# tspooner/rsrl

Hardware: AMD Instinct MI355X
Metric: env-steps/sec (whole node), MountainCar Q-learning Fourier-5 (higher is better)
Workload: dtype f32

## Files before the change

### rsrl_amd/csrc/abi_ctx.hip

```cpp
#include "ctx.hpp"

thread_local std::string g_last_error;

int fail(int code, const char* fmt, ...) {
    char buf[512];
    va_list ap; va_start(ap, fmt); vsnprintf(buf, sizeof(buf), fmt, ap); va_end(ap);
    g_last_error = buf;
    if (code == RSRL_HIP_EHIP || code == RSRL_HIP_ENOMEM) (void)hipGetLastError();
    return code;
}

static Switches read_switches() {
    Switches sw;
    sw.no_graph = getenv("RSRL_NO_GRAPH") != nullptr;
    sw.no_persist = getenv("RSRL_NO_PERSIST") != nullptr;
    sw.no_trait_defer = getenv("RSRL_NO_TRAIT_DEFER") != nullptr;
    sw.k1_feature_major = getenv("RSRL_K1_FEATURE_MAJOR") != nullptr;
    if (const char* e = getenv("RSRL_K1_QUAD")) sw.k1_quad = e[0] != '0' ? 1 : 0;
    if (const char* e = getenv("RSRL_SPARSE_CHUNK")) { const int v = atoi(e); sw.sparse_chunk = v > 0 && v < 16 ? 16 : v; }
    if (const char* e = getenv("RSRL_PEER_TIMEOUT_MS")) sw.peer_timeout_ms = atol(e);
    if (const char* e = getenv("RSRL_WAVE_PK")) sw.no_wave_pk = e[0] == '0';
    if (const char* e = getenv("RSRL_REG_PRODUCER")) sw.no_reg_producer = e[0] == '0';
    return sw;
}
bool no_coalesce_switch() { return getenv("RSRL_NO_COALESCE") != nullptr; }

static AgentFamily classify(const rsrl_hip_config& cfg, size_t w_elems) {
    using F = AgentFamily;
    const bool fourier = cfg.basis == RSRL_FOURIER, tile = cfg.basis == RSRL_TILE_CODING;
    const bool wave = is_wave(cfg), reg = is_reg_fourier(cfg);
    const int al = cfg.algo;
    if (cfg.domain == RSRL_HIV_TREATMENT) return F::Hiv;
    if (is_ac(al)) return F::AcReg;
    if (is_tdac(al)) return F::TdAcReg;
    if (is_reinforce(al)) return F::ReinforceReg;
    if (is_lstd(al)) return F::LstdReg;
    if (is_tdac_lstd(al)) return F::TdAcLstdReg;
    if (cfg.weight_mode == RSRL_W_SHARED) return fourier ? F::SharedDense : (is_sparse_lambda(cfg) ? F::SharedSparseLambda : F::SharedTile);
    if (wave && is_wave_aux_algo(al)) return F::WaveAux;
    if (is_pred(al)) return tile ? F::TdTile : (reg ? F::TdReg : F::TdGeneric);
    if (al == RSRL_Q_SIGMA) return wave ? F::WaveQSigma : (reg ? F::QSigmaReg : F::QSigmaGeneric);
    if (al == RSRL_GREEDY_GQ) return reg ? F::GqReg : F::GqGeneric;
    if (is_lambda(al)) return tile ? F::LambdaTile : (wave ? F::WaveLambda : (reg ? F::LambdaReg : F::LambdaGeneric));
    if (wave) return F::WaveControl;
    if (reg) return cfg.steps_per_launch == 1 && (uint64_t)w_elems * 4ull < (1ull << 32) ? F::RegStep : F::RegFused;
    return F::Generic;
}
static const char* train_kernel_name(const rsrl_hip_ctx* c) {
    if (c->family == AgentFamily::WaveControl && c->cfg.weight_dtype == RSRL_W_BF16 && !c->sw.no_wave_pk) return "k_train_wave_pk";
    if (c->family == AgentFamily::RegStep && c->w_ls != 1) return c->k1_quad ? "k_step_reg_q4" : "k_step_reg_lm";
    return family_row(c).kernel;
}
static size_t stat_slots(Slots geometry, int64_t N, int F) {
    switch (geometry) {
    case Slots::Block: return grid_for(N);
// ... 155 lines not shown
    TRY(check_config(*cfg));
    c->cfg = *cfg;
    c->D = kDomainShape[cfg->domain][0]; c->A = kDomainShape[cfg->domain][1];
    c->F = 1;
    for (int i = 0; i < c->D; ++i) c->F *= cfg->basis == RSRL_FOURIER ? cfg->order + 1 : cfg->tiles_per_dim;
    if (cfg->basis == RSRL_TILE_CODING) c->F *= cfg->n_tilings;
    int ndev = 0;
    HIP_TRY(hipGetDeviceCount(&ndev));
    if (ndev < 1) return fail(RSRL_HIP_EHIP, "no HIP device");
    if (cfg->device < 0 || cfg->device >= ndev) return fail(RSRL_HIP_EINVAL, "device %d out of range (%d devices)", cfg->device, ndev);
    HIP_TRY(hipSetDevice(cfg->device));
    { int cus = 0; HIP_TRY(hipDeviceGetAttribute(&cus, hipDeviceAttributeMultiprocessorCount, cfg->device)); if (cus > 0) { c->n_simd = 4 * cus; c->n_cu = cus; } }
    if (cfg->peer_timeout_ms < 0) return fail(RSRL_HIP_EINVAL, "peer_timeout_ms must be >= 0");
    c->sw = read_switches();
    if (cfg->peer_timeout_ms > 0) c->peer_timeout = (uint64_t)cfg->peer_timeout_ms * 100000ull;
    else if (c->sw.peer_timeout_ms > 0) c->peer_timeout = (uint64_t)c->sw.peer_timeout_ms * 100000ull;
    if (cfg->stream) { c->stream = (hipStream_t)cfg->stream; c->own_stream = false; }
    else { HIP_TRY(hipStreamCreateWithFlags(&c->stream, hipStreamNonBlocking)); c->own_stream = true; }
    const int64_t N = cfg->n_envs;
    const bool shared = cfg->weight_mode == RSRL_W_SHARED;
    c->w_stride = shared ? 1 : N;
    const AlgoRow& agent = kAlgo[cfg->algo];
    c->Aw = agent.v ? 1 : c->A;
    c->w_elems = (size_t)c->Aw * c->F * (size_t)(shared ? 1 : N);
    c->family = classify(*cfg, c->w_elems);
    if (c->family == AgentFamily::RegStep && (c->A * c->F) % 4 == 0 && c->F % 4 == 0 && !c->sw.k1_feature_major) {
        c->w_stride = 1;
        c->w_ls = (int64_t)c->A * c->F;
        c->k1_quad = c->A <= 3 && (c->sw.k1_quad >= 0 ? c->sw.k1_quad == 1 : N >= 131072);
    }
    if (c->family == AgentFamily::RegFused && !c->sw.no_reg_producer && cfg->epsilon_decay == 1.0 && N <= (int64_t)kBlock * c->n_cu) {
        int lds = 0;
        HIP_TRY(hipDeviceGetAttribute(&lds, hipDeviceAttributeMaxSharedMemoryPerBlock, cfg->device));
        c->reg_producer = train_reg_pw_serves(cfg->domain, cfg->order, cfg->algo, lds);
    }
    c->train_kernel = train_kernel_name(c);
    c->dw_elems = (size_t)c->Aw * c->F;
    c->n_stat_slots = stat_slots(c->k1_quad ? Slots::Block64 : family_row(c).slots, N, c->F);
    TRY(ctx_alloc(c, &c->state, sizeof(float) * c->D * (size_t)N));
    TRY(ctx_alloc(c, &c->action, sizeof(int32_t) * (size_t)N));
    TRY(ctx_alloc(c, &c->ep_step, sizeof(uint32_t) * (size_t)N));
    c->w_bytes = c->w_elems * (cfg->weight_dtype == RSRL_W_BF16 ? 2 : 4);
    TRY(ctx_alloc(c, &c->W, c->w_bytes));
    TRY(ctx_alloc(c, &c->dW, sizeof(float) * c->dw_elems));
    TRY(ctx_alloc(c, &c->qcache, sizeof(float) * c->A * (size_t)N));
    if (cfg->domain == RSRL_HIV_TREATMENT) TRY(ctx_alloc(c, &c->hiv_y, sizeof(double) * 6 * (size_t)N));
    if (c->w_ls != 1 && cfg->weight_dtype == RSRL_W_F32 && cfg->epsilon_decay == 1.0 && trait_lm_available(cfg->domain, cfg->order, cfg->algo)) {
        TRY(ctx_alloc(c, &c->tq_key, sizeof(float) * c->D * (size_t)N));
        TRY(ctx_alloc(c, &c->tq_q, sizeof(float) * c->A * (size_t)N));
    }
    if (cfg->algo == RSRL_Q_SIGMA) {
        TRY(ctx_alloc(c, &c->qs_buf, sizeof(float) * (size_t)(c->D + 5) * (size_t)cfg->n_steps * (size_t)N, true));
        TRY(ctx_alloc(c, &c->qs_head, sizeof(uint32_t) * (size_t)N, true));
        TRY(ctx_alloc(c, &c->qs_len, sizeof(uint32_t) * (size_t)N, true));
    }
    if (cfg->epsilon_decay != 1.0) {
        TRY(ctx_alloc(c, &c->eps, sizeof(float) * (size_t)N));
        hipLaunchKernelGGL(k_fill_f32, dim3(grid_for(N)), dim3(kBlock), 0, c->stream, c->eps, N, (float)cfg->epsilon);
        KCHECK();
    }
    if (c->family == AgentFamily::SharedSparseLambda) {
        const int64_t slice = (int64_t)(c->F / cfg->n_tilings) * c->A;
        if (slice > 65536) return fail(RSRL_HIP_EINVAL, "SARSALambda / QLambda over a shared tile table: one tiling's slice (cells * actions = %lld entries) must not "
                                                        "exceed 65 536 (16-bit slice-relative keys between the step and the trace kernel)", (long long)slice);
        TRY(ctx_alloc(c, &c->sp_len, sizeof(uint32_t) * (size_t)cfg->n_tilings * (size_t)N, true));
        TRY(ctx_alloc(c, &c->sp_keys, sizeof(uint16_t) * (size_t)kSparseCap * (size_t)N, true));
        TRY(ctx_alloc(c, &c->sp_vals, sizeof(float) * (size_t)kSparseCap * (size_t)N, true));
// ... 285 lines not shown
```

### rsrl_amd/csrc/abi_train.hip

```cpp
#include "ctx.hpp"

RSRL_DEFINE_FX_READER(fx_saturations_train)

int timing_begin(rsrl_hip_ctx* c) {
    if (!c->timing) return RSRL_HIP_OK;
    if (c->events_used == c->events.size()) {
        hipEvent_t a, b;
        HIP_TRY(hipEventCreate(&a)); HIP_TRY(hipEventCreate(&b));
        c->events.emplace_back(a, b);
    }
    HIP_TRY(hipEventRecord(c->events[c->events_used].first, c->stream));
    return RSRL_HIP_OK;
}
int timing_end(rsrl_hip_ctx* c, uint32_t launches) {
    if (!c->timing) return RSRL_HIP_OK;
    HIP_TRY(hipEventRecord(c->events[c->events_used].second, c->stream));
    if (c->event_launches.size() <= c->events_used) c->event_launches.resize(c->events_used + 1);
    c->event_launches[c->events_used] = launches;
    c->events_used++;
    return RSRL_HIP_OK;
}

static inline int fold_in_step(const rsrl_hip_ctx* c) { return !c->multi ? 1 : (c->cfg.exchange == RSRL_EXCHANGE_PEER ? 0 : 1); }
static inline long long* tab_set_of(const rsrl_hip_ctx* c, uint64_t t) { return c->sh_tab + (size_t)kTabRep * c->dw_elems * (size_t)(t % 3u); }
// ... 268 lines not shown
    const dim3 grid(grid_for(io ? io->M : k.n_envs)), block(kBlock);
    const bool td_lambda = cf.algo == RSRL_TD_LAMBDA;
    bool ok = true;
    switch (c->family) {
    case AgentFamily::WaveAux: case AgentFamily::WaveQSigma: case AgentFamily::WaveLambda:
        launch_wave_agent(c, k, t, chunk, d_stats, io); break;
    case AgentFamily::TdTile: ok = launch_td_tile(cf.domain, cf.n_tilings, td_lambda, c->stream, k, g, make_td(c), t, chunk, d_stats, io); break;
    case AgentFamily::TdGeneric: ok = launch_td_model(cf, grid, block, c->stream, k, make_td(c), g, td_lambda, t, chunk, d_stats, io); break;
    case AgentFamily::TdReg: ok = launch_td(cf.domain, cf.order, td_lambda, grid, block, c->stream, k, make_td(c), t, chunk, d_stats, io); break;
    case AgentFamily::QSigmaReg: ok = launch_qsigma(cf.domain, cf.order, grid, block, c->stream, k, make_qs(c), g, t, chunk, d_stats, io); break;
    case AgentFamily::QSigmaGeneric: ok = launch_qsigma_model(cf, grid, block, c->stream, k, make_qs(c), g, t, chunk, d_stats, io); break;
    case AgentFamily::GqReg: ok = launch_gq(cf.domain, cf.order, cf.policy, grid, block, c->stream, k, make_gq(c), t, chunk, d_stats, io); break;
    case AgentFamily::GqGeneric: ok = launch_gq_model(cf, grid, block, c->stream, k, make_gq(c), g, t, chunk, d_stats, io); break;
    case AgentFamily::LambdaTile: ok = launch_lambda_tile(cf.domain, cf.n_tilings, c->stream, k, g, make_lambda(c), t, chunk, d_stats, io); break;
    case AgentFamily::LambdaGeneric: ok = launch_lambda_model(cf, grid, block, c->stream, k, make_lambda(c), g, t, chunk, d_stats, io); break;
    case AgentFamily::LambdaReg: ok = launch_lambda(cf.domain, cf.order, cf.algo, cf.policy, grid, block, c->stream, k, make_lambda(c), t, chunk, d_stats, io); break;
    case AgentFamily::WaveControl:
        for_wave(c, [&](auto tag) {
            using T = decltype(tag); using WT = typename T::wt;
            const dim3 wg(wave_grid_for(k.n_envs));
            if constexpr (WaveIO<WT>::kBf16) {
                if (!c->sw.no_wave_pk) {
                    if (k.eps) hipLaunchKernelGGL((k_train_wave_pk<T::domain, true>), wg, block, 0, c->stream, k, (WT*)c->W, t, chunk, d_stats);
                    else hipLaunchKernelGGL((k_train_wave_pk<T::domain>), wg, block, 0, c->stream, k, (WT*)c->W, t, chunk, d_stats);
                    return;
                }
            }
            if (k.eps) hipLaunchKernelGGL((k_train_wave<T::domain, WT, true>), wg, block, 0, c->stream, k, (WT*)c->W, t, chunk, d_stats);
            else hipLaunchKernelGGL((k_train_wave<T::domain, WT>), wg, block, 0, c->stream, k, (WT*)c->W, t, chunk, d_stats);
        });
        break;
    case AgentFamily::RegStep: return enqueue_k1_step(c, k, d_stats, t, nullptr);
    case AgentFamily::RegFused:
        if (c->reg_producer && !k.eps) { ok = launch_train_reg_pw(cf.algo, cf.policy, grid, c->stream, k, t, chunk, d_stats); break; }
        ok = launch_train_reg(cf.domain, cf.order, cf.algo, cf.policy, grid, block, c->stream, k, t, chunk, d_stats);
        break;
    case AgentFamily::Generic:
        ok = for_model(c, [&](auto tag) {
            using M = typename decltype(tag)::type;
            hipLaunchKernelGGL((k_train_mem<M>), grid, block, 0, c->stream, k, g, t, chunk, d_stats);
        });
        break;
    case AgentFamily::Hiv:
        if (io) launch_hiv_handle(c->stream, k, g, *io, t);
        else launch_hiv_train(c->stream, k, g, c->hiv_y, t, chunk, d_stats);
        break;
    case AgentFamily::AcReg:
        ok = launch_ac(cf.domain, cf.order, cf.algo == RSRL_Q_ACTOR_CRITIC ? AC_CRITIC_Q : AC_CRITIC_ADVANTAGE, grid, block, c->stream, k, c->Z, t, chunk, d_stats, io);
        break;
    case AgentFamily::TdAcReg: ok = launch_tdac(cf.domain, cf.order, grid, block, c->stream, k, c->Z, t, chunk, d_stats, io); break;
    case AgentFamily::LstdReg: ok = launch_lstd(cf.domain, cf.order, cf.algo == RSRL_ILSTD, c->stream, k, make_lstd(c), t, chunk, d_stats, io); break;
    case AgentFamily::TdAcLstdReg: ok = launch_tdac_lstd(cf.domain, cf.order, c->stream, k, make_tdac_lstd(c), t, chunk, d_stats, io); break;
    case AgentFamily::ReinforceReg:
        ok = !io && launch_reinforce(cf.domain, cf.order, cf.algo == RSRL_BASELINE_REINFORCE, grid, block, c->stream, k, make_reinforce(c), t, chunk, d_stats, nullptr);
        break;
    default: ok = false; break;
    }
    if (!ok) return NO_MODEL(c);
    KCHECK();
    return RSRL_HIP_OK;
}

int train_now(rsrl_hip_ctx* c, int64_t n_steps, rsrl_hip_stats* stats_out) {
    HIP_TRY(hipSetDevice(c->cfg.device));
    c->tq_valid = false;
    DevStats* d_stats = stats_out ? c->d_stats : nullptr;
    if (d_stats) HIP_TRY(hipMemsetAsync(c->d_stats, 0, sizeof(DevStats) * c->n_stat_slots, c->stream));
// ... 182 lines not shown
```

### rsrl_amd/csrc/ctx.hpp

```cpp
#pragma once
#include <hip/hip_runtime.h>
#include <rccl/rccl.h>

#include <cmath>
#include <cstdarg>
#include <cstdio>
#include <cstring>
#include <unistd.h>
#include <dlfcn.h>
#include <map>
#include <mutex>
#include <string>
#include <vector>

#include "../../include/rsrl_hip.h"
#pragma GCC visibility push(hidden)
#define RSRL_API_BEGIN _Pragma("GCC visibility push(default)") extern "C" {
#define RSRL_API_END } _Pragma("GCC visibility pop")
#include "launch.hpp"
#include "models.hpp"
#include "model_list.hpp"
#include "kernels_wave.hpp"
#include "kernels_lambda.hpp"
#include "kernels_gq.hpp"
// ... 147 lines not shown
    {AgentFamily::GqGeneric, "k_train_gq_mem", 256, Slots::Block, Handle::Agent, 0},
    {AgentFamily::LambdaTile, "k_lambda_tile", 256, Slots::Learner, Handle::Agent, 0},
    {AgentFamily::WaveLambda, "k_wave_lambda", 256, Slots::WaveBlock, Handle::Agent, kWave},
    {AgentFamily::LambdaGeneric, "k_train_lambda_mem", 256, Slots::Block64, Handle::Agent, 0},
    {AgentFamily::LambdaReg, "k_train_lambda", 4096, Slots::Block, Handle::Agent, 0},
    {AgentFamily::WaveControl, "k_train_wave", 256, Slots::WaveBlock, Handle::Wave, kWave},
    {AgentFamily::RegStep, "k_step_reg", 4096, Slots::Block, Handle::Model, kCarriesQ},
    {AgentFamily::RegFused, "k_train_reg", 4096, Slots::Block, Handle::Model, kCarriesQ},
    {AgentFamily::Generic, "k_train_mem", 256, Slots::Block, Handle::Model, 0},
    {AgentFamily::Hiv, "k_hiv_train", 16, Slots::Block, Handle::Agent, 0},
    {AgentFamily::AcReg, "k_train_ac", 4096, Slots::Block, Handle::Agent, kPolicyW},
    {AgentFamily::TdAcReg, "k_train_tdac", 4096, Slots::Block, Handle::Agent, kPolicyW | kVCritic},
    {AgentFamily::ReinforceReg, "k_train_reinforce", 4096, Slots::Block, Handle::Agent, kPolicyW},
    {AgentFamily::LstdReg, "k_train_lstd", 32, Slots::LstdGroup, Handle::Agent, kLstd},
    {AgentFamily::TdAcLstdReg, "k_train_tdac_lstd", 32, Slots::LstdGroup, Handle::Agent, kPolicyW | kVCritic | kLstd},
};
constexpr bool family_rows_in_order() {
    for (size_t i = 0; i < sizeof(kFamily) / sizeof(kFamily[0]); ++i) if ((size_t)kFamily[i].family != i) return false;
    return true;
}
static_assert(sizeof(kFamily) / sizeof(kFamily[0]) == kAgentFamilies && family_rows_in_order(), "kFamily: one row per AgentFamily value, in the enum's order");
static inline bool is_wave_family(AgentFamily f) { return kFamily[(size_t)f].can & kWave; }

struct Switches {
    bool no_graph = false;
    bool no_persist = false;
    bool no_trait_defer = false;
    bool k1_feature_major = false;
    int k1_quad = -1;
    int sparse_chunk = 0;
    long peer_timeout_ms = 0;
    bool no_wave_pk = false;
    bool no_reg_producer = false;
};

struct rsrl_hip_ctx {
    rsrl_hip_config cfg{};
    AgentFamily family = AgentFamily::Generic;
    const char* train_kernel = "";
    Switches sw;
    int D = 0, A = 0, F = 0;
    hipStream_t stream = nullptr;
    bool own_stream = false;
    float* state = nullptr; int32_t* action = nullptr; uint32_t* ep_step = nullptr;
    float* W = nullptr; float* dW = nullptr;
    int Aw = 0;
    long long* dW_rep = nullptr; int n_rep = 1;
    long long* sh_tab = nullptr;
    long long* h_fx = nullptr;
    bool tile_slice = false;
    uint16_t* sc_keys = nullptr;
    float* sc_terms = nullptr;
    uint64_t sh_tab_t = 0;
    float* W2 = nullptr;
    int sh_par = 0;
    unsigned sh_rows = 0;
    float* qcache = nullptr;
    float* qs_buf = nullptr; uint32_t* qs_head = nullptr; uint32_t* qs_len = nullptr;
    float* eps = nullptr;
    uint16_t* sp_keys = nullptr; float* sp_vals = nullptr; uint32_t* sp_len = nullptr;
    bool sp_lds = false;
    float* Z = nullptr;
    float* Zb = nullptr;
    float* ret_g = nullptr;
    double* hiv_y = nullptr;
    double* lstd_theta = nullptr;
    double* lstd_mat = nullptr;
    double* lstd_mu = nullptr;
    bool q_valid = false;
    float* tq_key = nullptr;
    float* tq_q = nullptr;
    bool tq_valid = false;
    struct TraitPend { int stage = 0; const int32_t* act = nullptr; float* from = nullptr; float* to = nullptr; float* rew = nullptr;
                       uint8_t* term = nullptr; float* td = nullptr; uint64_t t_handle = 0; } tp;
    uint8_t* flags = nullptr;
    size_t w_elems = 0; size_t dw_elems = 0; size_t w_bytes = 0; size_t z_bytes = 0;
    int64_t w_stride = 0;
    int64_t w_ls = 1;
    DevStats* d_stats = nullptr; DevStats* h_stats = nullptr;
    size_t n_stat_slots = 0;
    bool k1_quad = false;
    bool reg_producer = false;
    uint64_t t = 0;
    int64_t pending = 0;
    uint64_t api_calls = 0;
    uint64_t rollout_calls = 0;
    Scratch scratch[8];
    std::vector<void**> owned;
    bool timing = false;
    std::vector<std::pair<hipEvent_t, hipEvent_t>> events;
    std::vector<uint32_t> event_launches;
    size_t events_used = 0;
    uint64_t* d_t = nullptr;
    DynParams* d_dyn = nullptr;
    DynParams dyn_uploaded{};
    bool dyn_valid = false;
    hipGraph_t step_graph = nullptr;
    hipGraphExec_t step_graph_exec = nullptr;
    Common step_graph_key{};
    int step_graph_kind = 0;
    const char* kernel_name = "";
    ncclComm_t comm = nullptr;
    int n_simd = 1024;
    int world_size = 1, rank = 0;
    bool multi = false;
    uint2* peer_recv = nullptr; size_t peer_recv_bytes = 0; int peer_world = 0;
    std::vector<void*> peer_ptrs; std::vector<char> peer_opened;
    uint2** d_peer_ptrs = nullptr;
    uint32_t* d_peer_err = nullptr;
    uint64_t peer_seq = 0;
    uint64_t peer_timeout = 400000000ull;
    size_t peer_old_bytes = 0;
    unsigned long long* px_A = nullptr; unsigned long long* px_B = nullptr; bool px_B_owned = false;
    unsigned long long** d_px_Bptrs = nullptr;
    uint64_t px_seq = 0;
// ... 301 lines not shown
```

### rsrl_amd/csrc/kernels_reg.hpp

```cpp
#pragma once

#include "device_core.hpp"

namespace rsrl {

struct DevStats {
    unsigned long long env_steps, episodes, episodes_truncated, sum_episode_steps;
    double sum_abs_td_error, sum_reward;
};

struct DynParams { PolicyParams pol, apol; };
struct Common {
    const DynParams* dyn;
    int64_t n_envs;
    int64_t env_offset;
    uint64_t seed;
    PolicyParams pol;
    PolicyParams apol;
    int apol_same;
    AlgoParams alg;
    uint32_t max_episode_steps;
    float* state;
    int32_t* action;
    uint32_t* ep_step;
// ... 286 lines not shown
        else if (q[i] > mx) { mx = q[i]; mask = (1u << i); }
    }
    mx_out = mx;
    return mask;
}
template <int A>
__device__ __forceinline__ float policy_eval_sa(const PolicyParams& pp, const float (&q)[A], int a) {
    if (pp.kind == POL_SOFTMAX) return select_a<A>(q, a);
    if (pp.kind == POL_RANDOM) return 1.0f / (float)A;
    float mx;
    const uint32_t mask = argmaxima_mask_max<A>(q, mx);
    const float pg = ((mask >> a) & 1u) ? 1.0f / (float)max(1, __popc(mask)) : 0.0f;
    if (pp.kind == POL_GREEDY) return pg;
    return pp.eps / (float)A + (1.0f - pp.eps) * pg;
}

template <int A>
__device__ __forceinline__ int find_min(const float (&q)[A], float& val) {
    int bi = 0; float bv = q[0];
#pragma unroll
    for (int i = 1; i < A; ++i) { if (!(bv < q[i])) { bi = i; bv = q[i]; } }
    val = bv;
    return bi;
}
template <int A>
__device__ __forceinline__ float expected_value(const float (&q)[A], const float (&p)[A]) {
    float acc = 0.0f;
#pragma unroll
    for (int i = 0; i < A; ++i) acc = acc + q[i] * p[i];
    return acc;
}


__device__ __forceinline__ const Common& step_common(const Common& c) { return c; }
__device__ __forceinline__ const Common& step_common(const Common* c) { return *c; }
template <int DOMAIN, int ORDER, int ALGO, int POLICY, bool ESCHED, bool STATS, int D, class Pre, int A, int F, bool PK, class C>
__device__ __forceinline__ auto reg_step(float (&s)[D], int& a, Pre& pre_s, uint32_t& ep, const uint32_t& cap, WBuf<A, F, PK>& w, QCarry& q_s, const AlgoParams& alg,
                                         PolicyParams& pol, const C& c, float& facc_abs, float& facc_r, uint32_t& n_ep, uint32_t& n_trunc) {
    using Dom = Domain<DOMAIN>;
    using Bas = FourierReg<DOMAIN, ORDER>;
    using Phi = PhiBuf<F, PK>;
    return [&](const Phi& phi_s, Phi& phi_n, const U4& x, const U4& xin) {
        float ns[D];
#pragma unroll
        for (int d = 0; d < D; ++d) ns[d] = s[d];
        float r;
        const bool term = Dom::step(ns, a, r, pre_s);
        ep += 1;
        const bool trunc = !term && cap > 0 && ep >= cap;
        if (term) Dom::reset(ns);
        pre_s = Dom::pre(ns);
        float q_n[A];
        { float ph[F]; Bas::project(ns, ph); phi_n.set(ph); }
        w.q(phi_n, q_n);
        static_assert(A <= 3, "ActionMask covers three actions");
        const ActionMask am(a);
        const float qsa = A > 2 ? bitsel(am.m2, q_s.v2, bitsel(am.m1, q_s.v1, q_s.v0)) : bitsel(am.m1, q_s.v1, q_s.v0);
        const float q_s_all[3] = {q_s.v0, q_s.v1, q_s.v2};
        float e;
        float delta;
        if constexpr (ALGO == ALG_PAL) {
            float qs_arr[A];
#pragma unroll
            for (int b = 0; b < A; ++b) qs_arr[b] = q_s_all[b];
            delta = td_error_pal<A>(alg, qs_arr, q_n, a, r, term, e);
        } else {
            delta = td_error_ap<A, ALGO>(alg, pol, step_common(c), qsa, q_n, r, term, xin, e);
        }
        const float scale = alg.lr * e;
        {
            float sb[A];
#pragma unroll
            for (int b = 0; b < A; ++b) sb[b] = and_mask(am.of(b), scale);
            w.axpy(sb, phi_s);
        }
        {
            const float dot = Phi::dot(phi_s, phi_n);
#pragma unroll
            for (int b = 0; b < A; ++b) q_n[b] = bitsel(am.of(b), fmaf(scale, dot, q_n[b]), q_n[b]);
        }
        if constexpr (ESCHED) learner_eps_step(step_common(c), term | trunc, pol);
        int na = policy_sample<A, true>(pol, q_n, x);
        if constexpr (STATS) {
            facc_abs += fabsf(delta);
            facc_r += r;
            n_ep += term ? 1u : 0u;
        }
        ep = term ? 0u : ep;
        if (__builtin_expect(trunc, 0)) {
            if constexpr (STATS) { n_ep += 1; n_trunc += 1; }
            ep = 0;
            Dom::reset(ns);
            pre_s = Dom::pre(ns);
            { float ph[F]; Bas::project(ns, ph); phi_n.set(ph); }
            w.q(phi_n, q_n);
            na = policy_sample<A, true>(pol, q_n, x);
        }
#pragma unroll
        for (int d = 0; d < D; ++d) s[d] = ns[d];
        q_s.set<A>(q_n);
        a = na;
    };
}

template <int DOMAIN, int ORDER, int ALGO, int POLICY, bool ESCHED = false>
__global__ __launch_bounds__(kBlock, 2) void k_train_reg(Common c, uint64_t t0, int n_steps, DevStats* __restrict__ stats) {
    using Dom = Domain<DOMAIN>;
    using Bas = FourierReg<DOMAIN, ORDER>;
    constexpr int D = Dom::D, A = Dom::A, F = Bas::F;
    const int64_t i = (int64_t)blockIdx.x * blockDim.x + threadIdx.x;
    const int64_t N = c.n_envs;
    char* __restrict__ const wblk = reinterpret_cast<char*>(c.W + (int64_t)blockIdx.x * blockDim.x * c.w_ls);
    const uint32_t wlane = threadIdx.x * (uint32_t)c.w_ls * 4u;
    const int64_t wrow = c.w_stride * 4;

    uint32_t n_ep = 0, n_trunc = 0, sum_len = 0;
    double sum_abs = 0.0, sum_r = 0.0;

    if (i < N) {
        PolicyParams pol = c.pol; pol.kind = POLICY;
        if constexpr (ESCHED) learner_eps_load(c, i, pol);
        AlgoParams alg = c.alg; alg.kind = ALGO;
        const uint32_t gid = (uint32_t)(c.env_offset + i);
        const uint32_t cap = c.max_episode_steps;
        float s[D];
#pragma unroll
        for (int d = 0; d < D; ++d) s[d] = c.state[(int64_t)d * N + i];
        int a = c.action[i];
        uint32_t ep = c.ep_step[i];
// ... 386 lines not shown
```

### rsrl_amd/csrc/kernels_reg_pw.hpp

```cpp
#pragma once

#include "kernels_reg.hpp"

namespace rsrl {
namespace pw {

constexpr int kConsumerWaves = kBlock / 64;
constexpr int kBlockPw = 2 * kBlock;
constexpr int kRingPairs = 8;
typedef uint32_t u4v __attribute__((ext_vector_type(4)));

constexpr size_t lds_bytes(bool inner) { return (size_t)kConsumerWaves * 2 * kRingPairs * (inner ? 2 : 1) * 64 * sizeof(u4v) + 512; }

constexpr int kGetregSimdId = 4 | (4 << 6) | (1 << 11);

__device__ __forceinline__ void block_stats_accumulate(DevStats* __restrict__ stats, bool consumer, int cw, unsigned long long n_ep,
                                                       unsigned long long n_trunc, unsigned long long sum_len, double sum_abs, double sum_r) {
    __shared__ unsigned long long sh_u[3][kConsumerWaves];
    __shared__ double sh_d[2][kConsumerWaves];
    n_ep = wave_sum(n_ep); n_trunc = wave_sum(n_trunc); sum_len = wave_sum(sum_len);
    sum_abs = wave_sum(sum_abs); sum_r = wave_sum(sum_r);
    if (consumer && (threadIdx.x & 63) == 0) {
        sh_u[0][cw] = n_ep; sh_u[1][cw] = n_trunc; sh_u[2][cw] = sum_len;
        sh_d[0][cw] = sum_abs; sh_d[1][cw] = sum_r;
    }
    __syncthreads();
    if (threadIdx.x == 0) {
        DevStats acc = stats[blockIdx.x];
        for (int w = 0; w < kConsumerWaves; ++w) {
            acc.episodes += sh_u[0][w]; acc.episodes_truncated += sh_u[1][w]; acc.sum_episode_steps += sh_u[2][w];
            acc.sum_abs_td_error += sh_d[0][w]; acc.sum_reward += sh_d[1][w];
        }
        stats[blockIdx.x] = acc;
    }
}

template <int DOMAIN, int ORDER, int ALGO, int POLICY, bool STATS = true>
__global__ __launch_bounds__(kBlockPw, 1) void k_train_reg(Common c, uint64_t t0, int n_steps, DevStats* __restrict__ stats) {
    using Dom = Domain<DOMAIN>;
    using Bas = FourierReg<DOMAIN, ORDER>;
    constexpr int D = Dom::D, A = Dom::A, F = Bas::F;
    constexpr bool INNER = ALGO == ALG_SARSA;
    constexpr int NS = INNER ? 2 : 1, H = kRingPairs;
    static_assert((H & (H - 1)) == 0, "ring slots are taken modulo 2H by a mask");
    __shared__ u4v ring[kConsumerWaves][2 * H][NS][64];
    __shared__ int claim[4];
    static_assert(sizeof(ring) + 512 == lds_bytes(INNER), "lds_bytes() is what the launcher checks against the device");

    const int lane = (int)(threadIdx.x & 63);
    const int wave = __builtin_amdgcn_readfirstlane((int)(threadIdx.x >> 6));
    if (threadIdx.x < 4) claim[threadIdx.x] = 0;
    __syncthreads();
    const int simd = (int)(__builtin_amdgcn_s_getreg(kGetregSimdId) & 3u);
    int slot = 0;
    if (lane == 0) slot = atomicAdd(&claim[simd], 1);
    __syncthreads();
    const int paired = __builtin_amdgcn_readfirstlane((claim[0] == 2 && claim[1] == 2 && claim[2] == 2 && claim[3] == 2) ? 1 : 0);
    slot = __builtin_amdgcn_readfirstlane(slot);
    const bool consumer = paired ? slot == 0 : wave < kConsumerWaves;
    const int cw = paired ? simd : (wave & (kConsumerWaves - 1));

    const int64_t N = c.n_envs;
    const int64_t blk0 = (int64_t)blockIdx.x * kBlock;
    const int64_t i = blk0 + cw * 64 + lane;
    const uint64_t th0 = t0 >> 1;
    const int NB = n_steps > 0 ? (int)(((t0 + (uint64_t)n_steps - 1) >> 1) - th0) + 1 : 0;
    const int G = (NB + H - 1) / H;

    uint32_t n_ep = 0, n_trunc = 0, sum_len = 0;
    double sum_abs = 0.0, sum_r = 0.0;

    if (!consumer) {
        const uint32_t gid = (uint32_t)(c.env_offset + i);
        for (int g = 0; g < G; ++g) {
            const int b1 = min((g + 1) * H, NB);
            for (int b = g * H; b < b1; ++b) {
                const U4 p = draw_block(c.seed, gid, th0 + (uint64_t)b, BLK_STEP);
                ring[cw][b & (2 * H - 1)][0][lane] = u4v{p.x, p.y, p.z, p.w};
                if constexpr (INNER) {
                    const U4 q = draw_block(c.seed, gid, th0 + (uint64_t)b, BLK_INNER);
                    ring[cw][b & (2 * H - 1)][NS - 1][lane] = u4v{q.x, q.y, q.z, q.w};
                }
            }
            __syncthreads();
        }
    } else {
        const bool valid = i < N;
        const int64_t il = valid ? i : N - 1;
        char* __restrict__ const wblk = reinterpret_cast<char*>(c.W + blk0 * c.w_ls);
        const uint32_t wlane = (uint32_t)(il - blk0) * (uint32_t)c.w_ls * 4u;
        const int64_t wrow = c.w_stride * 4;

        PolicyParams pol = c.pol; pol.kind = POLICY;
        AlgoParams alg = c.alg; alg.kind = ALGO;
        const uint32_t cap = c.max_episode_steps;
        float s[D];
#pragma unroll
        for (int d = 0; d < D; ++d) s[d] = c.state[(int64_t)d * N + il];
        int a = c.action[il];
        uint32_t ep = c.ep_step[il];
        const uint32_t ep_start = ep;
        constexpr bool PK = (RSRL_PK != 0) && (F % 4 == 0);
        using Phi = PhiBuf<F, PK>;
        WBuf<A, F, PK> w;
#pragma unroll
        for (int b = 0; b < A; ++b)
#pragma unroll
            for (int f = 0; f < F; ++f) w.put(b, f, row_load(wblk + (int64_t)(b * F + f) * wrow, wlane));

        static_assert(A <= 3, "QCarry holds up to 3 actions");
        Phi phi_a, phi_b;
        QCarry q_s;
        { float ph[F]; Bas::project(s, ph); phi_a.set(ph); }
        {
            float q0[A];
            if (c.q_valid) {
#pragma unroll
                for (int b = 0; b < A; ++b) q0[b] = c.qcache[(int64_t)b * N + il];
            } else {
                w.q(phi_a, q0);
            }
            q_s.set<A>(q0);
        }
        typename Dom::Pre pre_s = Dom::pre(s);
        float facc_abs = 0.0f, facc_r = 0.0f;
        __builtin_amdgcn_s_waitcnt(0x0070);

        const Common* const cs = ALGO != ALG_PAL ? &c : nullptr;
        const auto one_step = reg_step<DOMAIN, ORDER, ALGO, POLICY, false, STATS>(s, a, pre_s, ep, cap, w, q_s, alg, pol, cs, facc_abs, facc_r, n_ep, n_trunc);

        auto ring_read = [&](int b, int st) {
            const u4v v = ring[cw][b & (2 * H - 1)][st][lane];
            return U4{v.x, v.y, v.z, v.w};
        };
        const U4 zero4 = U4{0, 0, 0, 0};
        const bool lead = (t0 & 1u) && n_steps > 0;
        const bool trail = n_steps > 0 && ((t0 + (uint64_t)n_steps) & 1u);
        const int b_end = NB - (trail ? 1 : 0);

        __builtin_amdgcn_s_setprio(1);
        int b = 0;
        if (G > 0) __syncthreads();
        if (lead) {
            const U4 p = ring_read(0, 0), pin = INNER ? ring_read(0, NS - 1) : zero4;
            one_step(phi_a, phi_b, half_block(p, true), half_block(pin, true));
            const Phi tmp = phi_a; phi_a = phi_b; phi_b = tmp;
            b = 1;
        }
        for (int g = 0; g < G; ++g) {
            if (g > 0) __syncthreads();
            const int ge = min((g + 1) * H, b_end);
            if (b < ge) {
                U4 nx = ring_read(b, 0), nxin = INNER ? ring_read(b, NS - 1) : zero4;
                for (; b < ge; ++b) {
                    const U4 p = nx, pin = nxin;
                    const int bn = min(b + 1, ge - 1);
                    nx = ring_read(bn, 0);
                    if constexpr (INNER) nxin = ring_read(bn, NS - 1);
                    one_step(phi_a, phi_b, half_block(p, false), half_block(pin, false));
                    one_step(phi_b, phi_a, half_block(p, true), half_block(pin, true));
                }
            }
        }
        if (trail) {
            const U4 p = ring_read(NB - 1, 0), pin = INNER ? ring_read(NB - 1, NS - 1) : zero4;
            one_step(phi_a, phi_b, half_block(p, false), half_block(pin, false));
        }
        __builtin_amdgcn_s_setprio(0);

        if (valid) {
            sum_abs = (double)facc_abs; sum_r = (double)facc_r;
            sum_len = (uint32_t)n_steps + ep_start - ep;
#pragma unroll
            for (int d = 0; d < D; ++d) c.state[(int64_t)d * N + i] = s[d];
            c.action[i] = a;
            c.ep_step[i] = ep;
            c.qcache[i] = q_s.v0;
            if constexpr (A > 1) c.qcache[N + i] = q_s.v1;
            if constexpr (A > 2) c.qcache[2 * N + i] = q_s.v2;
            char* wblk_e = wblk;
            int64_t wrow_e = wrow;
            asm volatile("" : "+s"(wblk_e), "+s"(wrow_e));
#pragma unroll
            for (int bb = 0; bb < A; ++bb)
#pragma unroll
                for (int f = 0; f < F; ++f) row_store(wblk_e + (int64_t)(bb * F + f) * wrow_e, wlane, w.get(bb, f));
        } else {
            n_ep = 0; n_trunc = 0;
        }
    }

    if constexpr (STATS) {
        if (stats) block_stats_accumulate(stats, consumer, cw, n_ep, n_trunc, sum_len, sum_abs, sum_r);
    }
}

}
}
```

### rsrl_amd/csrc/launch.hpp

```cpp
#pragma once
#include "kernels_reg.hpp"
#include "kernels_reg_q4.hpp"

namespace rsrl {

bool launch_train_reg_d0(int order, int algo, int policy, dim3 grid, dim3 block, hipStream_t st,
                         const Common& k, uint64_t t, int chunk, DevStats* stats, const uint64_t* t_dev = nullptr);
bool launch_train_reg_d1(int order, int algo, int policy, dim3 grid, dim3 block, hipStream_t st,
                         const Common& k, uint64_t t, int chunk, DevStats* stats, const uint64_t* t_dev = nullptr);
bool launch_train_reg_d2(int order, int algo, int policy, dim3 grid, dim3 block, hipStream_t st,
                         const Common& k, uint64_t t, int chunk, DevStats* stats, const uint64_t* t_dev = nullptr);
static inline bool launch_train_reg(int domain, int order, int algo, int policy, dim3 grid, dim3 block, hipStream_t st,
                                    const Common& k, uint64_t t, int chunk, DevStats* stats, const uint64_t* t_dev = nullptr) {
    switch (domain) {
    case 0: return launch_train_reg_d0(order, algo, policy, grid, block, st, k, t, chunk, stats, t_dev);
    case 1: return launch_train_reg_d1(order, algo, policy, grid, block, st, k, t, chunk, stats, t_dev);
    default: return launch_train_reg_d2(order, algo, policy, grid, block, st, k, t, chunk, stats, t_dev);
    }
}

bool train_reg_pw_serves(int domain, int order, int algo, int lds_limit_bytes);
bool launch_train_reg_pw(int algo, int policy, dim3 grid, hipStream_t st, const Common& k, uint64_t t, int chunk, DevStats* stats);


struct Transitions {
    const float* from = nullptr; const int32_t* act = nullptr; const float* rew = nullptr; const float* to = nullptr; const uint8_t* term = nullptr;
    int64_t M = 0; float* td_out = nullptr;
};
static inline Transitions transitions_or_none(const Transitions* io) { return io ? *io : Transitions{}; }

struct LambdaParams;
struct BasisGeom;
bool launch_lambda(int domain, int order, int algo, int policy, dim3 grid, dim3 block, hipStream_t st, const Common& k, const LambdaParams& lp,
                   uint64_t t, int chunk, DevStats* stats, const Transitions* io);
bool launch_lambda_tile(int domain, int n_tilings, hipStream_t st, const Common& k, const BasisGeom& g, const LambdaParams& lp, uint64_t t, int chunk,
                        DevStats* stats, const Transitions* io);

struct TdParams;
bool launch_td_tile(int domain, int n_tilings, bool lambda, hipStream_t st, const Common& k, const BasisGeom& g, const TdParams& tp, uint64_t t, int chunk,
                    DevStats* stats, const Transitions* io);
bool launch_v_tile(int domain, int n_tilings, hipStream_t st, const Common& k, const BasisGeom& g, const float* states, int64_t M, float* out);

struct GqParams;
bool launch_gq(int domain, int order, int policy, dim3 grid, dim3 block, hipStream_t st, const Common& k, const GqParams& gp, uint64_t t, int chunk,
               DevStats* stats, const Transitions* io);

bool launch_ac(int domain, int order, int critic, dim3 grid, dim3 block, hipStream_t st, const Common& k, float* theta, uint64_t t, int chunk,
               DevStats* stats, const Transitions* io);
bool launch_tdac(int domain, int order, dim3 grid, dim3 block, hipStream_t st, const Common& k, float* theta, uint64_t t, int chunk, DevStats* stats,
                 const Transitions* io);
struct ReinforceState {
    float* theta = nullptr;
    float* theta_b = nullptr;
    float* g = nullptr;
};
// ... 91 lines not shown
```

### rsrl_amd/csrc/train_reg_pw.hip

```cpp
#include "launch.hpp"
#include "kernels_reg_pw.hpp"
namespace rsrl {
bool train_reg_pw_serves(int domain, int order, int algo, int lds_limit_bytes) {
    if (domain != 0 || order != 5) return false;
    if (algo != 0 && algo != 1 && algo != 2 && algo != 5) return false;
    return (size_t)(lds_limit_bytes > 0 ? lds_limit_bytes : 0) >= pw::lds_bytes(algo == ALG_SARSA);
}
#define RSRL_PW_CASE(AL, PO)                                                                                              \
    if (algo == AL && policy == PO) {                                                                                     \
        if (!stats)                     \
            hipLaunchKernelGGL((pw::k_train_reg<0, 5, AL, PO, false>), grid, dim3(pw::kBlockPw), 0, st, k, t, chunk, stats); \
        else                                                                                                              \
            hipLaunchKernelGGL((pw::k_train_reg<0, 5, AL, PO>), grid, dim3(pw::kBlockPw), 0, st, k, t, chunk, stats);     \
        return true;                                                                                                      \
    }
#define RSRL_PW_POLICIES(AL) RSRL_PW_CASE(AL, 0) RSRL_PW_CASE(AL, 1) RSRL_PW_CASE(AL, 2) RSRL_PW_CASE(AL, 3)
bool launch_train_reg_pw(int algo, int policy, dim3 grid, hipStream_t st, const Common& k, uint64_t t, int chunk, DevStats* stats) {
    RSRL_PW_POLICIES(0) RSRL_PW_POLICIES(1) RSRL_PW_POLICIES(2) RSRL_PW_POLICIES(5)
    return false;
}
}
```

Before: 73.08 billion.

## Digest random draws in producer waves and deepen the pw ring buffer

The producer waves of the producer/consumer RegFused kernel now pre-digest each Philox block into policy-specific values (epsilon masks, scaled uniforms, random action indices) before writing it to LDS. Consumer waves then do less arithmetic per step when sampling actions. For non-SARSA algorithms with enough LDS, the ring depth doubles from 8 to 16 pairs, and a full waitcnt is placed before the inner loop. The intent is to move sampling work off the critical consumer path and give producers more lead. The cost is more LDS use and more template instantiations.

```diff
diff --git a/rsrl_amd/csrc/abi_ctx.hip b/rsrl_amd/csrc/abi_ctx.hip
--- a/rsrl_amd/csrc/abi_ctx.hip
+++ b/rsrl_amd/csrc/abi_ctx.hip
@@ -21,6 +21,7 @@
     if (const char* e = getenv("RSRL_PEER_TIMEOUT_MS")) sw.peer_timeout_ms = atol(e);
     if (const char* e = getenv("RSRL_WAVE_PK")) sw.no_wave_pk = e[0] == '0';
     if (const char* e = getenv("RSRL_REG_PRODUCER")) sw.no_reg_producer = e[0] == '0';
+    if (const char* e = getenv("RSRL_REG_PW_RING")) sw.reg_pw_ring8 = atoi(e) == 8;
     return sw;
 }
 bool no_coalesce_switch() { return getenv("RSRL_NO_COALESCE") != nullptr; }
@@ -242,7 +243,7 @@
     if (c->family == AgentFamily::RegFused && !c->sw.no_reg_producer && cfg->epsilon_decay == 1.0 && N <= (int64_t)kBlock * c->n_cu) {
         int lds = 0;
         HIP_TRY(hipDeviceGetAttribute(&lds, hipDeviceAttributeMaxSharedMemoryPerBlock, cfg->device));
-        c->reg_producer = train_reg_pw_serves(cfg->domain, cfg->order, cfg->algo, lds);
+        c->reg_pw_ring = train_reg_pw_ring(cfg->domain, cfg->order, cfg->algo, lds, c->sw.reg_pw_ring8);
     }
     c->train_kernel = train_kernel_name(c);
     c->dw_elems = (size_t)c->Aw * c->F;
diff --git a/rsrl_amd/csrc/abi_train.hip b/rsrl_amd/csrc/abi_train.hip
--- a/rsrl_amd/csrc/abi_train.hip
+++ b/rsrl_amd/csrc/abi_train.hip
@@ -324,7 +324,7 @@
         break;
     case AgentFamily::RegStep: return enqueue_k1_step(c, k, d_stats, t, nullptr);
     case AgentFamily::RegFused:
-        if (c->reg_producer && !k.eps) { ok = launch_train_reg_pw(cf.algo, cf.policy, grid, c->stream, k, t, chunk, d_stats); break; }
+        if (c->reg_pw_ring && !k.eps) { ok = launch_train_reg_pw(cf.algo, cf.policy, c->reg_pw_ring, grid, c->stream, k, t, chunk, d_stats); break; }
         ok = launch_train_reg(cf.domain, cf.order, cf.algo, cf.policy, grid, block, c->stream, k, t, chunk, d_stats);
         break;
     case AgentFamily::Generic:
diff --git a/rsrl_amd/csrc/ctx.hpp b/rsrl_amd/csrc/ctx.hpp
--- a/rsrl_amd/csrc/ctx.hpp
+++ b/rsrl_amd/csrc/ctx.hpp
@@ -203,6 +203,7 @@
     long peer_timeout_ms = 0;
     bool no_wave_pk = false;
     bool no_reg_producer = false;
+    bool reg_pw_ring8 = false;
 };
 
 struct rsrl_hip_ctx {
@@ -251,7 +252,7 @@
     DevStats* d_stats = nullptr; DevStats* h_stats = nullptr;
     size_t n_stat_slots = 0;
     bool k1_quad = false;
-    bool reg_producer = false;
+    int reg_pw_ring = 0;
     uint64_t t = 0;
     int64_t pending = 0;
     uint64_t api_calls = 0;
diff --git a/rsrl_amd/csrc/kernels_reg.hpp b/rsrl_amd/csrc/kernels_reg.hpp
--- a/rsrl_amd/csrc/kernels_reg.hpp
+++ b/rsrl_amd/csrc/kernels_reg.hpp
@@ -342,6 +342,8 @@
 }
 
 
+template <int A>
+__device__ __forceinline__ int step_sample(const PolicyParams& pol, const float (&q)[A], const U4& x) { return policy_sample<A, true>(pol, q, x); }
 __device__ __forceinline__ const Common& step_common(const Common& c) { return c; }
 __device__ __forceinline__ const Common& step_common(const Common* c) { return *c; }
 template <int DOMAIN, int ORDER, int ALGO, int POLICY, bool ESCHED, bool STATS, int D, class Pre, int A, int F, bool PK, class C>
@@ -350,7 +352,7 @@
     using Dom = Domain<DOMAIN>;
     using Bas = FourierReg<DOMAIN, ORDER>;
     using Phi = PhiBuf<F, PK>;
-    return [&](const Phi& phi_s, Phi& phi_n, const U4& x, const U4& xin) {
+    return [&](const Phi& phi_s, Phi& phi_n, const auto& x, const auto& xin) {
         float ns[D];
 #pragma unroll
         for (int d = 0; d < D; ++d) ns[d] = s[d];
@@ -390,7 +392,7 @@
             for (int b = 0; b < A; ++b) q_n[b] = bitsel(am.of(b), fmaf(scale, dot, q_n[b]), q_n[b]);
         }
         if constexpr (ESCHED) learner_eps_step(step_common(c), term | trunc, pol);
-        int na = policy_sample<A, true>(pol, q_n, x);
+        int na = step_sample<A>(pol, q_n, x);
         if constexpr (STATS) {
             facc_abs += fabsf(delta);
             facc_r += r;
@@ -404,7 +406,7 @@
             pre_s = Dom::pre(ns);
             { float ph[F]; Bas::project(ns, ph); phi_n.set(ph); }
             w.q(phi_n, q_n);
-            na = policy_sample<A, true>(pol, q_n, x);
+            na = step_sample<A>(pol, q_n, x);
         }
 #pragma unroll
         for (int d = 0; d < D; ++d) s[d] = ns[d];
diff --git a/rsrl_amd/csrc/kernels_reg_pw.hpp b/rsrl_amd/csrc/kernels_reg_pw.hpp
--- a/rsrl_amd/csrc/kernels_reg_pw.hpp
+++ b/rsrl_amd/csrc/kernels_reg_pw.hpp
@@ -1,16 +1,15 @@
 #pragma once
 
 #include "kernels_reg.hpp"
+#include "reg_pw_ring.hpp"
 
 namespace rsrl {
 namespace pw {
 
-constexpr int kConsumerWaves = kBlock / 64;
+static_assert(kConsumerWaves == kBlock / 64, "four consumer waves: the learners of a block, as in k_train_reg");
 constexpr int kBlockPw = 2 * kBlock;
-constexpr int kRingPairs = 8;
 typedef uint32_t u4v __attribute__((ext_vector_type(4)));
-
-constexpr size_t lds_bytes(bool inner) { return (size_t)kConsumerWaves * 2 * kRingPairs * (inner ? 2 : 1) * 64 * sizeof(u4v) + 512; }
+static_assert(kSlotBytes == 64 * sizeof(u4v), "a ring slot: one Philox block per lane");
 
 constexpr int kGetregSimdId = 4 | (4 << 6) | (1 << 11);
 
@@ -35,17 +34,91 @@
     }
 }
 
-template <int DOMAIN, int ORDER, int ALGO, int POLICY, bool STATS = true>
+struct Digested { uint32_t x, y; };
+__device__ __forceinline__ uint32_t mad3_u24(uint32_t a, uint32_t c) {
+#if defined(__HIP_DEVICE_COMPILE__)
+    uint32_t r;
+    asm("v_mad_u32_u24 %0, %1, 3, %2" : "=v"(r) : "v"(a), "v"(c));
+    return r;
+#else
+    return a * 3u + c;
+#endif
+}
+template <int A>
+__device__ __forceinline__ U4 digest(const PolicyParams& pp, const U4& p) {
+#if defined(RSRL_PW_RAW_DRAWS)
+    return p;
+#else
+    switch (pp.kind) {
+    case POL_EGREEDY: { constexpr uint32_t full = (1u << A) - 1u; return U4{(p.x >> 8) < pp.eps_thr ? full : 0u, p.y, (p.z >> 8) < pp.eps_thr ? full : 0u, p.w}; }
+    case POL_SOFTMAX: return U4{p.x, __builtin_bit_cast(uint32_t, (float)(p.y >> 8) * (1.0f / 16777216.0f)), p.z,
+                                __builtin_bit_cast(uint32_t, (float)(p.w >> 8) * (1.0f / 16777216.0f))};
+    case POL_RANDOM: return U4{p.x, mulhi_u32(p.y, (uint32_t)A), p.z, mulhi_u32(p.w, (uint32_t)A)};
+    default: return p;
+    }
+#endif
+}
+template <int A>
+__device__ __forceinline__ int sample_digested(const PolicyParams& pp, const float (&q)[A], const Digested& d) {
+#if defined(RSRL_PW_RAW_DRAWS)
+    return policy_sample<A, true>(pp, q, U4{d.x, d.y, d.y, 0u});
+#else
+    switch (pp.kind) {
+    case POL_EGREEDY: {
+        constexpr uint32_t full = (1u << A) - 1u;
+        const uint32_t m0 = argmaxima_mask<A>(q);
+        const uint32_t mask = (m0 == 0u ? full : m0) | d.x;
+        static_assert(A == 3, "the table's row length");
+        return kth_set_bit<A>(0u, (int)mad3_u24(mask, mulhi_u32(d.y, (uint32_t)__popc(mask))));
+    }
+    case POL_SOFTMAX: {
+        float p[A]; softmax_probs<A>(q, pp.tau, p);
+        const float u = __builtin_bit_cast(float, d.y);
+        float acc = 0.0f; int res = A - 1; bool found = false;
+#pragma unroll
+        for (int i = 0; i < A; ++i) {
+            acc = acc + p[i];
+            if (!found && acc > u) { res = i; found = true; }
+        }
+        return res;
+    }
+    case POL_RANDOM: return (int)d.y;
+    default: return greedy_sample<A>(q, d.y);
+    }
+#endif
+}
+__device__ __forceinline__ Digested half_digested(const U4& p, bool odd) { return odd ? Digested{p.z, p.w} : Digested{p.x, p.y}; }
+
+template <int A>
+__device__ __forceinline__ int step_sample(const PolicyParams& pol, const float (&q)[A], const Digested& x) { return sample_digested<A>(pol, q, x); }
+template <int A, int ALGO>
+__device__ __forceinline__ float td_error_ap(const AlgoParams& alg, const PolicyParams& pol, const Common& c, float qsa, const float (&qn)[A], float r,
+                                             bool term, const Digested& xin, float& e) {
+    if constexpr (ALGO == ALG_SARSA) {
+        const int na = !c.apol_same ? sample_digested<A>(c.apol, qn, xin) : sample_digested<A>(pol, qn, xin);
+        float boot = qn[0];
+#pragma unroll
+        for (int i = 1; i < A; ++i) boot = (na == i) ? qn[i] : boot;
+        const float d_term = r - qsa, d_boot = r + alg.gamma * boot - qsa;
+        const float delta = term ? d_term : d_boot;
+        e = delta;
+        return delta;
+    } else {
+        return rsrl::td_error_ap<A, ALGO>(alg, pol, c, qsa, qn, r, term, U4{0, 0, 0, 0}, e);
+    }
+}
+
+template <int DOMAIN, int ORDER, int ALGO, int POLICY, bool STATS = true, int H = kRingPairs>
 __global__ __launch_bounds__(kBlockPw, 1) void k_train_reg(Common c, uint64_t t0, int n_steps, DevStats* __restrict__ stats) {
     using Dom = Domain<DOMAIN>;
     using Bas = FourierReg<DOMAIN, ORDER>;
     constexpr int D = Dom::D, A = Dom::A, F = Bas::F;
     constexpr bool INNER = ALGO == ALG_SARSA;
-    constexpr int NS = INNER ? 2 : 1, H = kRingPairs;
+    constexpr int NS = INNER ? 2 : 1;
     static_assert((H & (H - 1)) == 0, "ring slots are taken modulo 2H by a mask");
     __shared__ u4v ring[kConsumerWaves][2 * H][NS][64];
     __shared__ int claim[4];
-    static_assert(sizeof(ring) + 512 == lds_bytes(INNER), "lds_bytes() is what the launcher checks against the device");
+    static_assert(sizeof(ring) + 512 == lds_bytes(INNER, H), "lds_bytes() is what the launcher checks against the device");
 
     const int lane = (int)(threadIdx.x & 63);
     const int wave = __builtin_amdgcn_readfirstlane((int)(threadIdx.x >> 6));
@@ -72,13 +145,15 @@
 
     if (!consumer) {
         const uint32_t gid = (uint32_t)(c.env_offset + i);
+        PolicyParams pol = c.pol; pol.kind = POLICY;
+        const PolicyParams ipol = (INNER && !c.apol_same) ? c.apol : pol;
         for (int g = 0; g < G; ++g) {
             const int b1 = min((g + 1) * H, NB);
             for (int b = g * H; b < b1; ++b) {
-                const U4 p = draw_block(c.seed, gid, th0 + (uint64_t)b, BLK_STEP);
+                const U4 p = digest<A>(pol, draw_block(c.seed, gid, th0 + (uint64_t)b, BLK_STEP));
                 ring[cw][b & (2 * H - 1)][0][lane] = u4v{p.x, p.y, p.z, p.w};
                 if constexpr (INNER) {
-                    const U4 q = draw_block(c.seed, gid, th0 + (uint64_t)b, BLK_INNER);
+                    const U4 q = digest<A>(ipol, draw_block(c.seed, gid, th0 + (uint64_t)b, BLK_INNER));
                     ring[cw][b & (2 * H - 1)][NS - 1][lane] = u4v{q.x, q.y, q.z, q.w};
                 }
             }
@@ -143,7 +218,7 @@
         if (G > 0) __syncthreads();
         if (lead) {
             const U4 p = ring_read(0, 0), pin = INNER ? ring_read(0, NS - 1) : zero4;
-            one_step(phi_a, phi_b, half_block(p, true), half_block(pin, true));
+            one_step(phi_a, phi_b, half_digested(p, true), half_digested(pin, true));
             const Phi tmp = phi_a; phi_a = phi_b; phi_b = tmp;
             b = 1;
         }
@@ -152,19 +227,22 @@
             const int ge = min((g + 1) * H, b_end);
             if (b < ge) {
                 U4 nx = ring_read(b, 0), nxin = INNER ? ring_read(b, NS - 1) : zero4;
+#if !defined(RSRL_PW_LATE_WAIT)
+                __builtin_amdgcn_s_waitcnt(0xC07F);
+#endif
                 for (; b < ge; ++b) {
                     const U4 p = nx, pin = nxin;
                     const int bn = min(b + 1, ge - 1);
                     nx = ring_read(bn, 0);
                     if constexpr (INNER) nxin = ring_read(bn, NS - 1);
-                    one_step(phi_a, phi_b, half_block(p, false), half_block(pin, false));
-                    one_step(phi_b, phi_a, half_block(p, true), half_block(pin, true));
+                    one_step(phi_a, phi_b, half_digested(p, false), half_digested(pin, false));
+                    one_step(phi_b, phi_a, half_digested(p, true), half_digested(pin, true));
                 }
             }
         }
         if (trail) {
             const U4 p = ring_read(NB - 1, 0), pin = INNER ? ring_read(NB - 1, NS - 1) : zero4;
-            one_step(phi_a, phi_b, half_block(p, false), half_block(pin, false));
+            one_step(phi_a, phi_b, half_digested(p, false), half_digested(pin, false));
         }
         __builtin_amdgcn_s_setprio(0);
 
diff --git a/rsrl_amd/csrc/launch.hpp b/rsrl_amd/csrc/launch.hpp
--- a/rsrl_amd/csrc/launch.hpp
+++ b/rsrl_amd/csrc/launch.hpp
@@ -19,8 +19,8 @@
     }
 }
 
-bool train_reg_pw_serves(int domain, int order, int algo, int lds_limit_bytes);
-bool launch_train_reg_pw(int algo, int policy, dim3 grid, hipStream_t st, const Common& k, uint64_t t, int chunk, DevStats* stats);
+int train_reg_pw_ring(int domain, int order, int algo, int lds_limit_bytes, bool ring8);
+bool launch_train_reg_pw(int algo, int policy, int ring_pairs, dim3 grid, hipStream_t st, const Common& k, uint64_t t, int chunk, DevStats* stats);
 
 
 struct Transitions {
diff --git a/rsrl_amd/csrc/reg_pw_ring.hpp b/rsrl_amd/csrc/reg_pw_ring.hpp
--- /dev/null
+++ b/rsrl_amd/csrc/reg_pw_ring.hpp
@@ -0,0 +1,21 @@
+#pragma once
+#include <cstddef>
+
+namespace rsrl {
+namespace pw {
+
+constexpr int kConsumerWaves = 4;
+constexpr int kRingPairs = 8;
+constexpr int kRingPairsDeep = 16;
+constexpr size_t kSlotBytes = 16 * 64;
+
+constexpr size_t lds_bytes(bool inner, int H) { return (size_t)kConsumerWaves * 2 * H * (inner ? 2 : 1) * kSlotBytes + 512; }
+
+constexpr int ring_pairs(bool inner, long long lds_limit, bool ring8) {
+    const size_t lds = (size_t)(lds_limit > 0 ? lds_limit : 0);
+    if (!inner && !ring8 && lds >= lds_bytes(inner, kRingPairsDeep)) return kRingPairsDeep;
+    return lds >= lds_bytes(inner, kRingPairs) ? kRingPairs : 0;
+}
+
+}
+}
diff --git a/rsrl_amd/csrc/train_reg_pw.hip b/rsrl_amd/csrc/train_reg_pw.hip
--- a/rsrl_amd/csrc/train_reg_pw.hip
+++ b/rsrl_amd/csrc/train_reg_pw.hip
@@ -1,22 +1,23 @@
 #include "launch.hpp"
 #include "kernels_reg_pw.hpp"
 namespace rsrl {
-bool train_reg_pw_serves(int domain, int order, int algo, int lds_limit_bytes) {
-    if (domain != 0 || order != 5) return false;
-    if (algo != 0 && algo != 1 && algo != 2 && algo != 5) return false;
-    return (size_t)(lds_limit_bytes > 0 ? lds_limit_bytes : 0) >= pw::lds_bytes(algo == ALG_SARSA);
+int train_reg_pw_ring(int domain, int order, int algo, int lds_limit_bytes, bool ring8) {
+    if (domain != 0 || order != 5) return 0;
+    if (algo != 0 && algo != 1 && algo != 2 && algo != 5) return 0;
+    return pw::ring_pairs(algo == ALG_SARSA, lds_limit_bytes, ring8);
 }
-#define RSRL_PW_CASE(AL, PO)                                                                                              \
-    if (algo == AL && policy == PO) {                                                                                     \
+#define RSRL_PW_CASE(AL, PO, H)                                                                                           \
+    if (algo == AL && policy == PO && ring_pairs == H) {                                                                  \
         if (!stats)                     \
-            hipLaunchKernelGGL((pw::k_train_reg<0, 5, AL, PO, false>), grid, dim3(pw::kBlockPw), 0, st, k, t, chunk, stats); \
+            hipLaunchKernelGGL((pw::k_train_reg<0, 5, AL, PO, false, H>), grid, dim3(pw::kBlockPw), 0, st, k, t, chunk, stats); \
         else                                                                                                              \
-            hipLaunchKernelGGL((pw::k_train_reg<0, 5, AL, PO>), grid, dim3(pw::kBlockPw), 0, st, k, t, chunk, stats);     \
+            hipLaunchKernelGGL((pw::k_train_reg<0, 5, AL, PO, true, H>), grid, dim3(pw::kBlockPw), 0, st, k, t, chunk, stats);  \
         return true;                                                                                                      \
     }
-#define RSRL_PW_POLICIES(AL) RSRL_PW_CASE(AL, 0) RSRL_PW_CASE(AL, 1) RSRL_PW_CASE(AL, 2) RSRL_PW_CASE(AL, 3)
-bool launch_train_reg_pw(int algo, int policy, dim3 grid, hipStream_t st, const Common& k, uint64_t t, int chunk, DevStats* stats) {
-    RSRL_PW_POLICIES(0) RSRL_PW_POLICIES(1) RSRL_PW_POLICIES(2) RSRL_PW_POLICIES(5)
+#define RSRL_PW_POLICIES(AL, H) RSRL_PW_CASE(AL, 0, H) RSRL_PW_CASE(AL, 1, H) RSRL_PW_CASE(AL, 2, H) RSRL_PW_CASE(AL, 3, H)
+bool launch_train_reg_pw(int algo, int policy, int ring_pairs, dim3 grid, hipStream_t st, const Common& k, uint64_t t, int chunk, DevStats* stats) {
+    RSRL_PW_POLICIES(0, pw::kRingPairs) RSRL_PW_POLICIES(1, pw::kRingPairs) RSRL_PW_POLICIES(2, pw::kRingPairs) RSRL_PW_POLICIES(5, pw::kRingPairs)
+    RSRL_PW_POLICIES(0, pw::kRingPairsDeep) RSRL_PW_POLICIES(2, pw::kRingPairsDeep) RSRL_PW_POLICIES(5, pw::kRingPairsDeep)
     return false;
 }
 }
```

New measurement: 73.70 billion (median of 4 runs). About the same (+0.9%).
